# nikitakaraevv/ray-tracing-engine

Hardware: AMD Instinct MI355X
Metric: Mrays/s (primary+secondary) at 1024x1024/128spp path trace (higher is better)
Workload: dtype f32

## Files before the change

### include/rt_pixelmode.h

```cpp
#ifndef RT_PIXELMODE_H
#define RT_PIXELMODE_H

#include <stdint.h>
#include <string.h>

#if defined(__HIPCC__)
#define RT_HD __host__ __device__ inline
#else
#define RT_HD static inline
#endif

#define RT_STREAM_PIXEL 0u
#define RT_STREAM_PHOTON 1u
#define RT_STREAM_AO 2u
#define RT_STREAM_LENS 3u
#define RT_STREAM_SHUTTER 4u
#define RT_STREAM_PICK 5u

RT_HD uint64_t rt_mix64(uint64_t z) {
  z ^= z >> 30;
  z *= 0xbf58476d1ce4e5b9ull;
  z ^= z >> 27;
  z *= 0x94d049bb133111ebull;
  z ^= z >> 31;
// ... 19 lines not shown
  memcpy(&d, &u, 8);
  return d;
}

RT_HD double rt_pow2(double x) { return x * x; }
RT_HD double rt_pow5(double x) {
  double x2 = x * x;
  return (x2 * x2) * x;
}

#if defined(__HIP_DEVICE_COMPILE__)
RT_HD double rt_sqrt_d(double x) { return __dsqrt_rn(x); }
#else
RT_HD double rt_sqrt_d(double x) { return __builtin_sqrt(x); }
#endif

RT_HD double rt_asin_poly(double t) {
  const double pS0 = 1.66666666666666657415e-01, pS1 = -3.25565818622400915405e-01,
               pS2 = 2.01212532134862925881e-01, pS3 = -4.00555345006794114027e-02,
               pS4 = 7.91534994289814532176e-04, pS5 = 3.47933107596021167570e-05,
               qS1 = -2.40339491173441421878e+00, qS2 = 2.02094576023350569471e+00,
               qS3 = -6.88283971605453293030e-01, qS4 = 7.70381505559019352791e-02;
  double p = t * (pS0 + t * (pS1 + t * (pS2 + t * (pS3 + t * (pS4 + t * pS5)))));
  double q = 1.0 + t * (qS1 + t * (qS2 + t * (qS3 + t * qS4)));
  return p / q;
}

RT_HD double rt_asin(double x) {
  const double pio2_hi = 1.57079632679489655800e+00, pio2_lo = 6.12323399573676603587e-17,
               pio4_hi = 7.85398163397448278999e-01;
  double ax = x < 0.0 ? -x : x;
  if (!(ax <= 1.0)) return rt_u2d(0x7ff8000000000000ull);
  if (ax == 1.0) return x * pio2_hi + x * pio2_lo;
  if (ax < 0.5) {
    if (ax < 7.450580596923828125e-09) return x;
    return x + x * rt_asin_poly(x * x);
  }
  double w = 1.0 - ax;
  double t = w * 0.5;
  double r = rt_asin_poly(t);
  double s = rt_sqrt_d(t);
  double res;
  if (ax >= 0.975) {
    res = pio2_hi - (2.0 * (s + s * r) - pio2_lo);
  } else {
    double sh = rt_u2d(rt_d2u(s) & 0xffffffff00000000ull);
    double c = (t - sh * sh) / (s + sh);
    double p = 2.0 * s * r - (pio2_lo - 2.0 * c);
    double q = pio4_hi - 2.0 * sh;
    res = pio4_hi - (p - q);
  }
  return x < 0.0 ? -res : res;
}

RT_HD double rt_ksin(double r) {
  const double S1 = -1.66666666666666324348e-01, S2 = 8.33333333332248946124e-03,
               S3 = -1.98412698298579493134e-04, S4 = 2.75573137070700676789e-06,
               S5 = -2.50507602534068634195e-08, S6 = 1.58969099521155010221e-10;
  double z = r * r;
  double v = z * r;
  double p = S2 + z * (S3 + z * (S4 + z * (S5 + z * S6)));
  return r + v * (S1 + z * p);
}
RT_HD double rt_kcos(double r) {
  const double C1 = 4.16666666666666019037e-02, C2 = -1.38888888888741095749e-03,
               C3 = 2.48015872894767294178e-05, C4 = -2.75573143513906633035e-07,
               C5 = 2.08757232129817482790e-09, C6 = -1.13596475577881948265e-11;
  double z = r * r;
  double p = z * (C1 + z * (C2 + z * (C3 + z * (C4 + z * (C5 + z * C6)))));
  return 1.0 - (0.5 * z - z * p);
}
RT_HD double rt_reduce_pio2(float xf, int* quadrant) {
  const double invpio2 = 6.36619772367581382433e-01, pio2_1 = 1.57079632673412561417e+00,
// ... 43 lines not shown
```

### ray-tracing-engine_amd/csrc/rt_api.cpp

```cpp
#include <hip/hip_runtime.h>

#include <dlfcn.h>
#include <rccl/rccl.h>

#include <algorithm>
#include <chrono>
#include <cmath>
#include <map>
#include <memory>
#include <mutex>
#include <cstdarg>
#include <cstdio>
#include <cstdlib>
#include <cstring>
#include <initializer_list>
#include <string>
#include <thread>
#include <type_traits>
#include <vector>

#include "bvh_build.h"
#include "filters.h"
#include "rt_amd.h"
#include "rt_kernels.h"

namespace {

thread_local std::string g_err;

int fail(int code, const char* fmt, ...) {
  char buf[512];
  va_list ap;
  va_start(ap, fmt);
  vsnprintf(buf, sizeof buf, fmt, ap);
  va_end(ap);
  g_err = buf;
  return code;
}

#define HIP_TRY(expr)                                                                      \
  do {                                                                                     \
    hipError_t e_ = (expr);                                                                \
    if (e_ != hipSuccess) return fail(RT_ERR_HIP, "%s failed: %s", #expr, hipGetErrorString(e_)); \
  } while (0)

int select_device(int device) {
  int n = 0;
  hipError_t e = hipGetDeviceCount(&n);
  if (e != hipSuccess || n <= 0)
    return fail(RT_ERR_NO_DEVICE, "no HIP device available (%s); this library has no CPU path",
                e == hipSuccess ? "device count is 0" : hipGetErrorString(e));
  if (device < 0 || device >= n) return fail(RT_ERR_NO_DEVICE, "device %d out of range (0..%d)", device, n - 1);
  hipDeviceProp_t prop;
  HIP_TRY(hipGetDeviceProperties(&prop, device));
  if (strncmp(prop.gcnArchName, "gfx950", 6) != 0)
    return fail(RT_ERR_NO_DEVICE, "device %d is %s; kernels are built for gfx950 only", device, prop.gcnArchName);
  HIP_TRY(hipSetDevice(device));
// ... 120 lines not shown
    return RT_OK;
  }
};

struct StreamList {
  DevBuf<uint32_t> d;
  PinnedBuf<uint32_t> h;
  Event ready;
  hipStream_t on = nullptr;
  uint32_t n = 0;
};
int stream_upload(StreamList* L, const std::vector<uint32_t>& v, hipStream_t stream) {
  L->n = 0;
  if (L->d) {
    HIP_TRY(hipEventSynchronize(L->ready.get()));
    HIP_TRY(hipFree(L->d.release()));
  }
  L->h.reset();
  if (v.empty()) return RT_OK;
  HIP_TRY(dev_alloc(&L->d, v.size()));
  HIP_TRY(pinned_alloc(&L->h, v.size()));
  memcpy(L->h.get(), v.data(), v.size() * sizeof(uint32_t));
  if (!L->ready) HIP_TRY(make_event(&L->ready, hipEventDisableTiming));
  HIP_TRY(hipMemcpyAsync(L->d.get(), L->h.get(), v.size() * sizeof(uint32_t), hipMemcpyHostToDevice, stream));
  HIP_TRY(hipEventRecord(L->ready.get(), stream));
  L->on = stream, L->n = static_cast<uint32_t>(v.size());
  return RT_OK;
}
int use_on(const StreamList& L, hipStream_t stream) {
  if (L.d && stream != L.on) HIP_TRY(hipStreamWaitEvent(stream, L.ready.get(), 0));
  return RT_OK;
}

struct TileKey {
  uint32_t w = 0, h = 0, rank = 0, world = 0, tile = 0, sshift = 0;
  bool operator==(const TileKey& o) const {
    return w == o.w && h == o.h && rank == o.rank && world == o.world && tile == o.tile && sshift == o.sshift;
  }
};

void wave_tile_shape(uint32_t sshift, uint32_t& tw, uint32_t& th) {
  static const uint32_t W[7] = {8, 8, 4, 4, 2, 2, 1}, H[7] = {8, 4, 4, 2, 2, 1, 1};
  tw = W[sshift], th = H[sshift];
}

constexpr int kEventPairs = 256;

}

struct rt_ctx {
  int device = 0;
  rtk::DevScene S{};
  rtbvh::Built bvh;
  DevBuf<uint4> triShade, nodes, q8;
  DevBuf<float> vpos, vnrm;
  DevBuf<float4> tris, trisRef;
  DevBuf<rt_material> mats;
  DevBuf<rtd::DevMat> matsDev;
  DevBuf<rt_light> lights;
  DevBuf<uint32_t> meshTriBegin, meshVtxBegin;
  DevBuf<float4> nodesF;
  DevBuf<float4> phPos, phDir;
  DevBuf<uint4> phTopo;
  StreamList tiles;
  TileKey tileKey;
  DevBuf<unsigned long long> dCounters;
  DevBuf<uint32_t> dTileCounter;
  using GranList = StreamList;
  std::map<std::string, GranList> granules;
  rtk::WfArgs wf{};
  size_t wfCap = 0;
  DevBuf<char> wfBlock;
  uint32_t builder = RT_BVH_HOST;
  bool broken = false;
  uint32_t recipCheck = 0;
  uint32_t nodeFormat = RT_NODES_F16;
  float buildMs = 0.f;
  uint32_t numCUs = 0;
  Event ev[kEventPairs][2];
  int evUsed = 0;
  std::vector<rt_light> hostLights;
  uint32_t nMeshes = 0, nVertices = 0;
  uint32_t magRef = 0, magPos = 0, magNrm = 0;
  DevBuf<uint8_t> refitDepth;
  uint32_t refitMaxDepth = 0;
  uint32_t optLeafMax = 0, optBuilder = RT_BVH_AUTO, optNodeFormat = RT_NODES_AUTO;
  double costBuilt = 0.0;
  bool costBuiltValid = false;
  uint32_t refits = 0;
  DevBuf<double> dQuality;
  DevBuf<float> updPos, updNrm;
  DevBuf<uint32_t> dMag;
  DevBuf<float> restPos, restNrm;
  bool restValid = false;
  DevBuf<rt_mesh_transform> xfTable;
  DevBuf<uint16_t> skinBone;
  DevBuf<float> skinWeight;
  DevBuf<rt_mesh_transform> skinTable;
// ... 60 lines not shown
void install_photons(rt_ctx* c, DevBuf<float4> pos, DevBuf<float4> dir, DevBuf<uint4> topo, uint32_t n) {
  c->phPos = std::move(pos), c->phDir = std::move(dir), c->phTopo = std::move(topo);
  c->S.phPos = c->phPos.get(), c->S.phDir = c->phDir.get(), c->S.phTopo = c->phTopo.get(), c->S.n_photons = n;
}
uint32_t photons_per_light(uint32_t n_requested, uint32_t n_lights) {
  const float lightPdf = 1.f / static_cast<float>(n_lights);
  return static_cast<uint32_t>(static_cast<int>(static_cast<float>(static_cast<int>(n_requested)) * lightPdf));
}

uint32_t choose_sshift_px(const rt_ctx* c, const rt_params* p, uint64_t pixels, uint32_t spp_count, bool pick = false) {
  if (p->reserved[0]) {
    uint32_t s = 0;
    while ((1u << (s + 1)) <= p->reserved[0] && s < 6) ++s;
    return s;
  }
  const uint64_t target = 32ull * 256 * 16;
  uint32_t s = 0;
  while (s < 6 && (pixels << s) / 64 < target && (2u << s) <= spp_count) ++s;
  const bool pooled = !p->use_photons && p->accel != RT_ACCEL_BRUTE && (pick || c->S.n_lights <= 3u) && !(p->reserved[1] & 1u) &&
                      !(p->reserved[2] & 1u);
  if (pooled) {
    const uint32_t want = c->S.n_nodes > 65536u ? 6u : 4u;
    while (s < want && (2u << s) <= spp_count) ++s;
  }
  if (p->use_photons && p->accel != RT_ACCEL_BRUTE)
    while (s < 6u && (2u << s) <= spp_count) ++s;
  return s;
}
uint32_t choose_sshift(const rt_ctx* c, const rt_params* p, uint32_t spp_count, bool pick = false) {
  const uint64_t world = p->world ? p->world : 1;
  return choose_sshift_px(c, p, (uint64_t)p->width * p->height / world, spp_count, pick);
}

template <class F>
void owned_granules(uint32_t w, uint32_t h, uint32_t rank, uint32_t world, uint32_t tile, F f) {
  if (tile == 0) tile = 8;
  if (world == 0) world = 1;
  const uint32_t gx = (w + 7) / 8, gy = (h + 7) / 8;
  for (uint32_t y8 = 0; y8 < gy; ++y8)
    for (uint32_t x8 = 0; x8 < gx; ++x8)
      if (world <= 1 || (x8 * 8 / tile + y8 * 8 / tile) % world == rank) f(x8, y8);
}

TileKey tile_key(const rt_params* p, uint32_t sshift) {
  TileKey k;
  k.w = p->width, k.h = p->height, k.rank = p->rank, k.world = p->world ? p->world : 1;
  k.tile = p->tile ? p->tile : 8;
  k.sshift = sshift;
  return k;
}
std::vector<uint32_t> wave_tiles(const TileKey& k) {
  std::vector<uint32_t> tiles;
  uint32_t tw, th;
  wave_tile_shape(k.sshift, tw, th);
  owned_granules(k.w, k.h, k.rank, k.world, k.tile, [&](uint32_t x8, uint32_t y8) {
    for (uint32_t y = y8 * 8; y < y8 * 8 + 8 && y < k.h; y += th)
      for (uint32_t x = x8 * 8; x < x8 * 8 + 8 && x < k.w; x += tw) tiles.push_back(x | (y << 16));
  });
  return tiles;
}

int ensure_tiles(rt_ctx* c, const rt_params* p, uint32_t sshift, hipStream_t stream) {
  const TileKey k = tile_key(p, sshift);
  if (c->tiles.d && k == c->tileKey) return use_on(c->tiles, stream);
  const int rc = stream_upload(&c->tiles, wave_tiles(k), stream);
  if (rc != RT_OK) return rc;
  c->tileKey = k;
  return RT_OK;
}

int ensure_granules(rt_ctx* c, const rt_params* p, uint32_t rank, hipStream_t stream, const rt_ctx::GranList** out) {
  char key[96];
  snprintf(key, sizeof key, "%u.%u.%u.%u.%u", p->width, p->height, rank, p->world ? p->world : 1, p->tile ? p->tile : 8);
  auto it = c->granules.find(key);
  if (it == c->granules.end()) {
    std::vector<uint32_t> g;
    owned_granules(p->width, p->height, rank, p->world, p->tile, [&](uint32_t x8, uint32_t y8) { g.push_back(x8 | (y8 << 16)); });
    rt_ctx::GranList L;
    int rc = stream_upload(&L, g, stream);
    if (rc != RT_OK) return rc;
    it = c->granules.emplace(key, std::move(L)).first;
  } else {
    const int rc = use_on(it->second, stream);
    if (rc != RT_OK) return rc;
  }
  *out = &it->second;
  return RT_OK;
}

int check_params_shape(const rt_params* p) {
  if (p->width == 0 || p->height == 0 || p->width > 65535u || p->height > 65535u)
    return fail(RT_ERR_INVALID, "image size %ux%u out of range", p->width, p->height);
  if (p->spp == 0) return fail(RT_ERR_INVALID, "spp must be >= 1");
  if (p->mode != RT_MODE_RAY && p->mode != RT_MODE_PATH) return fail(RT_ERR_INVALID, "mode must be 0 or 1");
  if (p->rng_mode != RT_RNG_PIXEL)
    return fail(RT_ERR_UNSUPPORTED,
                "rng_mode legacy is one global serial engine (reference LightSource.h:6) and cannot run in "
                "parallel; the GPU path implements RT_RNG_PIXEL only");
  if (p->max_depth < 1 || p->max_depth > 3) return fail(RT_ERR_UNSUPPORTED, "max_depth must be in 1..3");
  if (p->world > 1 && p->rank >= p->world) return fail(RT_ERR_INVALID, "rank %u >= world %u", p->rank, p->world);
  if (p->tile % 8 != 0) return fail(RT_ERR_INVALID, "tile must be a multiple of 8");
// ... 110 lines not shown
    W.col = reinterpret_cast<float4*>(take(P * 48));
    W.org = reinterpret_cast<float4*>(take(P * 16)), W.dir = reinterpret_cast<float4*>(take(P * 16));
    W.nrm = reinterpret_cast<float4*>(take(P * 16)), W.pnt = reinterpret_cast<float4*>(take(P * 16));
    W.res = reinterpret_cast<uint2*>(take(P * 32)), W.key = reinterpret_cast<uint2*>(take(P * 8));
    W.rng = reinterpret_cast<uint32_t*>(take(P * 4));
    W.stripes = reinterpret_cast<unsigned long long*>(take(2048 * sizeof(unsigned long long)));
    const hipError_t he = hipMemsetAsync(W.stripes, 0, 2048 * sizeof(unsigned long long), stream);
    if (he != hipSuccess) {
      c->wfCap = 0;
      return fail(RT_ERR_HIP, "wavefront stripes reset failed: %s", hipGetErrorString(he));
    }
  }
  rtk::WfArgs W = c->wf;
  W.gran = G->d.get(), W.nGran = G->n, W.width = p->width, W.height = p->height, W.spp = p->spp, W.seed = p->seed;
  W.s0 = A.s0, W.s1 = A.s1, W.batch = (uint32_t)batch, W.nPaths = 0;
  *out = W;
  return RT_OK;
}

struct TileList {
  const uint32_t* tiles;
  uint32_t n, sshift;
  const uint32_t* tileView = nullptr;
  const rtk::ViewRec* views = nullptr;
  const rtk::ViewShutterRec* viewShutters = nullptr;
};

using FrameGen = rtk::FrameVariant;

int launch_frame(rt_ctx* c, const rt_params* p, float4* dAccum, hipStream_t stream, int* evIndex,
                 const TileList* own = nullptr, const FrameGen& gen = FrameGen()) {
  const SampleRange sr = sample_range(*p);
  const uint32_t sshift = own ? own->sshift : choose_sshift(c, p, sr.count, gen.kind == FrameGen::PICK);
  int rc = own ? RT_OK : ensure_tiles(c, p, sshift, stream);
  if (rc != RT_OK) return rc;
  rtk::RenderArgs A;
  A.sshift = sshift;
  wave_tile_shape(sshift, A.tileW, A.tileH);
  A.tiles = own ? own->tiles : c->tiles.d.get(), A.n_tiles = own ? own->n : c->tiles.n;
  A.tileView = own ? own->tileView : nullptr, A.views = own ? own->views : nullptr;
  A.viewShutters = own ? own->viewShutters : nullptr;
  A.width = p->width, A.height = p->height, A.spp = p->spp;
  A.s0 = sr.s0, A.s1 = sr.s1;
  A.mode = p->mode, A.max_depth = p->max_depth, A.seed = p->seed;
  A.k = p->k, A.photons_requested = p->photons_requested;
  static const bool noPool = getenv("RT_NO_POOL") != nullptr;
  A.flags = (noPool || (p->reserved[1] & 1u)) ? 0u : 1u;
  if (c->bvh.leafMax <= 2u) A.flags |= 2u;
  uint32_t levels = c->bvh.maxDepth > 1 ? c->bvh.maxDepth : 1;
  A.kd16 = 0;
  if (p->use_photons) {
    const KdStack ks = kd_stack(c->S.n_photons);
    A.kd16 = ks.kd16 ? 1u : 0u;
    levels = levels > ks.rows ? levels : ks.rows;
  }
  A.stackLevels = stack_levels(levels);
  A.tileCounter = c->dTileCounter.get(), A.numCUs = c->numCUs, A.waveWords = 0, A.tilesPerBlock = 1;
  const bool wavefront = (p->reserved[2] & 1u) && !p->use_photons && p->accel != RT_ACCEL_BRUTE && c->S.n_lights <= 3u;
  rtk::WfArgs W{};
  if (wavefront && (rc = wavefront_args(c, p, A, sr.count, stream, &W)) != RT_OK) return rc;
  return timed_launch(c, stream, evIndex, [&] {
    if (const FrameGen V = A.viewShutters ? FrameGen(FrameGen::VIEWS_SHUTTER) : gen) {
      hipError_t he = rtk::launch_render_variant(V, p->accel == RT_ACCEL_BRUTE, p->collect_stats != 0, c->S, A, dAccum,
                                                 c->dCounters.get(), stream);
      if (he != hipSuccess) return fail(RT_ERR_HIP, "%s render launch failed: %s", V.name(), hipGetErrorString(he));
    } else if (!wavefront) {
      hipError_t he = rtk::launch_render(p->accel == RT_ACCEL_BRUTE, p->use_photons != 0, p->collect_stats != 0, c->S, A,
                                         dAccum, c->dCounters.get(), stream);
      if (he != hipSuccess) return fail(RT_ERR_HIP, "render launch failed: %s", hipGetErrorString(he));
    } else if (W.nGran) {
      hipError_t hw = rtk::launch_wavefront(c->S, W, p->mode, p->max_depth, dAccum, c->dCounters.get(), c->dTileCounter.get(),
                                            A.stackLevels, c->numCUs, stream);
      if (hw != hipSuccess) return fail(RT_ERR_HIP, "wavefront launch failed: %s", hipGetErrorString(hw));
    }
    return (int)RT_OK;
  });
}

}

extern "C" {

int rt_abi_version(void) { return RT_ABI_VERSION; }
const char* rt_last_error(void) { return g_err.c_str(); }

}

namespace {
int create_ctx(const rt_scene_desc* sc, const rt_options* opt, const rtbvh::Built* prebuilt, rt_ctx** out);
}

// ... 3318 lines not shown
```

### ray-tracing-engine_amd/csrc/rt_kernels.h

```cpp
#pragma once

#include <hip/hip_runtime.h>
#include <stdint.h>

#include "bvh_build.h"
#include "rt_amd.h"
#include "rt_device.h"

#define RTK_KMAX 16

enum {
  RTK_CNT_CLOSEST = 0,
  RTK_CNT_SHADOW,
  RTK_CNT_KNN,
  RTK_CNT_NODES,
  RTK_CNT_TRIS,
  RTK_CNT_KD,
  RTK_CNT_WNODE,
  RTK_CNT_WLEAF,
  RTK_CNT_LWAIT,
  RTK_CNT_LIDLE,
  RTK_CNT_FRAMES,
  RTK_CNT_COUNT = 32
};
// ... 32 lines not shown
struct ViewRec {
  rt_camera cam;
  uint32_t seed;
  uint32_t accumOff;
  uint32_t pad[2];
};
static_assert(sizeof(ViewRec) == 64, "ViewRec is four 16-byte scalar loads");

struct ViewShutterRec {
  float d[12];
  float open, close;
  float aperture;
  float fs0, dfs;
  uint32_t pad[3];
};
static_assert(sizeof(ViewShutterRec) == 80 && sizeof(ViewShutterRec) % 16 == 0, "ViewShutterRec is five 16-byte scalar loads");

struct RenderArgs {
  const uint32_t* tiles;
  uint32_t n_tiles;
  uint32_t width, height, spp, s0, s1, mode, max_depth, seed, k, photons_requested;
  uint32_t flags;
  uint32_t stackLevels;
  uint32_t kd16;
  uint32_t sshift;
  uint32_t tileW, tileH;
  uint32_t tilesPerBlock;
  uint32_t* tileCounter;
  uint32_t waveWords;
  uint32_t numCUs;
  const uint32_t* tileView;
  const ViewRec* views;
  const ViewShutterRec* viewShutters;
};

hipError_t launch_render(bool brute_force, bool photon, bool stats, const DevScene& S, const RenderArgs& A,
                         float4* accum, unsigned long long* counters, hipStream_t stream);
hipError_t launch_resolve(uint32_t n_pixels, uint32_t spp, const float4* accum, const float* bg, float* out,
                          hipStream_t stream);
struct WfArgs {
  const uint32_t* gran;
  uint32_t nGran, width, height, spp, seed;
  uint32_t s0, s1;
  uint32_t batch;
  uint32_t nPaths;
  uint32_t* rng;
  float4 *org, *dir;
  uint2* key;
  float4 *nrm, *pnt;
  float4* col;
  float4 *rayO, *rayD;
  uint2* res;
  unsigned long long* stripes;
};
hipError_t launch_wavefront(const DevScene& S, const WfArgs& W, uint32_t mode, uint32_t maxDepth, float4* accum,
                            unsigned long long* counters, uint32_t* queueCounter, uint32_t stackLevels, uint32_t numCUs,
                            hipStream_t stream);
struct TexDesc;
struct TexRec;
struct AovArgs {
  float *albedo, *normal, *position, *depth;
  uint32_t *hits, *mesh, *tri;
  uint32_t width, height, spp, seed, s0, s1;
  const ViewRec* views = nullptr;
  uint32_t tilesPerView = 0;
  const float* vcol = nullptr;
  const float* texUv = nullptr;
  const uint32_t* texMesh = nullptr;
// ... 168 lines not shown
```

### ray-tracing-engine_amd/csrc/rt_kernels.hip

```cpp
#include <hip/hip_runtime.h>

#include <cstdio>
#include <cstdlib>
#include <type_traits>

#include "bvh_build.h"
#include "filters.h"
#include "rt_device.h"
#include "rt_kernels.h"

using namespace rtd;

namespace rtk {

constexpr int BLOCK = 64;
constexpr int STACK = rtbvh::kMaxDepth;
constexpr int KMAX = RTK_KMAX;

struct Lds {
  uint32_t* stack;
  uint2* heap;
};

#ifdef RT_PHASE_TIMING
// ... 1092 lines not shown
  wave_sync();
  if (owner) {
    const uint32_t cnt = A.s1 - base < S_ ? A.s1 - base : S_;
#pragma unroll
    for (int g = 0; g < RT_LIGHT_GROUPS_MAX; ++g) {
      if ((uint32_t)g < G.n) {
        float4 s = accum[g * slice + pix];
        for (uint32_t jj = 0; jj < cnt; jj++) {
          const uint32_t q = jj * P_ + pl;
          s.x += ex[(3 * g + 0) * 64 + q], s.y += ex[(3 * g + 1) * 64 + q], s.z += ex[(3 * g + 2) * 64 + q];
          s.w += ex[HIT + q];
        }
        accum[g * slice + pix] = s;
      }
    }
  }
  wave_sync();
}

struct NoRec {};
template <int LTV>
using frame_rec_t = std::conditional_t<(LTV & LT_LENS) != 0, LensRec,
                    std::conditional_t<(LTV & LT_LIGHTS) != 0, LightGroupsRec,
                    std::conditional_t<(LTV & LT_PICK) != 0, PickRec,
                    std::conditional_t<(LTV & LT_VCOL) != 0, VColRec,
                    std::conditional_t<(LTV & LT_TEX) != 0, TexRec,
                    std::conditional_t<(LTV & LT_SHUTTER) != 0 && (LTV & LT_VIEWS) == 0, ShutterRec, NoRec>>>>>>;
template <int LTV>
constexpr const frame_rec_t<LTV>* no_record() {
  static_assert(std::is_same_v<frame_rec_t<LTV>, NoRec>, "this variant's instances pass their record to render_tile");
  return nullptr;
}

template <bool BRUTE, bool PHOTON, bool POOLED, bool STATS, int LTV, class HP = Heap>
RT_DEV void render_tile(const DevScene& S, const RenderArgs& A, float4* __restrict__ accum, const Lds& L, uint32_t* pool,
                        float* ex, uint32_t wave, LaneStats& st, const frame_rec_t<LTV>* rec = no_record<LTV>(),
                        float* park = nullptr) {
  constexpr int LT = LTV & ~(LT_VIEWS | LT_LENS | LT_SHUTTER | LT_LIGHTS | LT_PICK | LT_VCOL | LT_TEX);
  constexpr bool VIEWS = (LTV & LT_VIEWS) != 0;
  constexpr bool LENS = (LTV & LT_LENS) != 0;
  constexpr bool SHUTTER = (LTV & LT_SHUTTER) != 0;
  constexpr bool LIGHTS = (LTV & LT_LIGHTS) != 0;
  constexpr bool PICK = (LTV & LT_PICK) != 0;
  constexpr bool VCOL = (LTV & LT_VCOL) != 0;
  constexpr bool TEX = (LTV & LT_TEX) != 0;
  static_assert(!VCOL || (!VIEWS && !LENS && !SHUTTER && !LIGHTS && !PICK && !PHOTON), "vertex colours go with the plain frame only");
  static_assert(!TEX || (!VIEWS && !LENS && !SHUTTER && !LIGHTS && !PICK && !VCOL && !PHOTON), "textures go with the plain frame only");
  static_assert(!LIGHTS || (!VIEWS && !LENS && !SHUTTER && !PHOTON), "light groups go with the plain frame only");
  static_assert(!PICK || (!VIEWS && !LENS && !SHUTTER && !LIGHTS && !PHOTON), "light picks go with the plain frame only");
  static_assert(!LENS || !VIEWS, "no multi-view lens frames");
  static_assert(!SHUTTER || !LENS, "the shutter's lens is its own: LT_SHUTTER does not go with LT_LENS");
  constexpr bool FR = (LT & LT_FASTDET) != 0;
  const uint32_t lane = threadIdx.x & 63u;
  const uint32_t tile = A.tiles[wave];
  rt_camera cam;
  uint32_t seed = A.seed;
  ShutterRec vsh;
  if constexpr (VIEWS) {
    typedef const __attribute__((address_space(4))) uint32_t* const_u32_ptr;
    typedef const __attribute__((address_space(4))) ViewRec* const_view_ptr;
    typedef const __attribute__((address_space(4))) ViewShutterRec* const_shutter_ptr;
    const uint32_t view = ((const_u32_ptr)A.tileView)[wave];
    const const_view_ptr R = (const_view_ptr)A.views + view;
    for (int j = 0; j < 3; ++j)
      cam.position[j] = R->cam.position[j], cam.lower_left[j] = R->cam.lower_left[j],
      cam.horizontal[j] = R->cam.horizontal[j], cam.vertical[j] = R->cam.vertical[j];
    seed = R->seed;
    accum += R->accumOff;
    if constexpr (SHUTTER) {
      const const_shutter_ptr Q = (const_shutter_ptr)A.viewShutters + view;
      for (int j = 0; j < 12; ++j) vsh.d[j] = Q->d[j];
      vsh.open = Q->open, vsh.close = Q->close, vsh.aperture = Q->aperture, vsh.fs0 = Q->fs0, vsh.dfs = Q->dfs;
    }
  }
  const uint32_t S_ = 1u << A.sshift, P_ = 64u >> A.sshift;
  const uint32_t pl = lane & (P_ - 1u), sj = lane >> (6u - A.sshift);
  const uint32_t wsh = (uint32_t)__builtin_ctz(A.tileW);
  const uint32_t px = (tile & 0xffffu) + (pl & (A.tileW - 1u)), py = (tile >> 16) + (pl >> wsh);
  const bool inImage = px < A.width && py < A.height;
  const bool owner = inImage && sj == 0;
  const uint32_t pix = inImage ? py * A.width + px : 0u;
  float4 sum = owner ? accum[pix] : make_float4(0.f, 0.f, 0.f, 0.f);
  constexpr bool pooled = POOLED;
  const int nvert = A.mode == RT_MODE_PATH ? (int)A.max_depth : 1;
  for (uint32_t base = A.s0; base < A.s1; base += S_) {
    const uint32_t i = base + sj;
    const bool active = inImage && i < A.s1;
    Rng g{rt_stream_seed(VIEWS ? seed : A.seed, RT_STREAM_PIXEL, pix, i)};
    float sx, sy;
    jitter_sample(g, (int)i, (int)A.spp, sx, sy);
    f3 o, d;
    const float cu = ((float)px + sx) / (float)A.width, cv = 1.f - ((float)py + sy) / (float)A.height;
    if constexpr (VIEWS && SHUTTER) shutter_ray(cam, vsh, seed, pix, i, cu, cv, o, d);
    else if constexpr (VIEWS) camera_ray<FR>(cam, cu, cv, o, d);
    else if constexpr (LENS) {
      if (rec->aperture > 0.f) lens_ray(S.cam, *rec, rt_stream_seed(A.seed, RT_STREAM_LENS, pix, i), cu, cv, o, d);
      else camera_ray<FR>(S.cam, cu, cv, o, d);
    } else if constexpr (SHUTTER) shutter_ray(S.cam, *rec, A.seed, pix, i, cu, cv, o, d);
    else camera_ray<FR>(S.cam, cu, cv, o, d);
    f3 c0 = mk(0.f, 0.f, 0.f), c1 = c0, c2 = c0;
    GroupCols g0, g1, g2, gv;
    if constexpr (LIGHTS) group_cols_zero(g0), group_cols_zero(g1), group_cols_zero(g2);
    bool primary = true, alive = active;
    Picks pk{0u, 0u, 0u};
    if constexpr (PICK) pk = draw_picks(*rec, A.seed, pix, i);
    if constexpr (pooled) {
      HitRec h;
      if (alive) st.closest++;
      const bool hit0 = cast<false, false, STATS, LT>(S, alive, o, d, L.stack, h, st);
      if (alive && !hit0) primary = false, alive = false;
      for (int depth = 0; depth < nvert; depth++) {
// ... 71 lines not shown
        if (alive)
          c = shade_direct_seq<BRUTE, STATS, false, NoPick, VColKd>(S, g, d, h, L.stack, nrm, pt, st, nullptr, nullptr, NoPick(),
                                                                    VColKd{vertex_kd(S, rec->vcol, S.triShade[h.id], h.u, h.v), park});
      } else if constexpr (TEX) {
        if (alive)
          c = shade_direct_seq<BRUTE, STATS, false, NoPick, VColKd>(S, g, d, h, L.stack, nrm, pt, st, nullptr, nullptr, NoPick(),
                                                                    VColKd{tex_kd(S, *rec, S.triShade[h.id], h.u, h.v), park});
      } else {
        if (alive) c = shade_direct_seq<BRUTE, STATS>(S, g, d, h, L.stack, nrm, pt, st);
      }
      if (alive) {
        if (depth == 0) c0 = c;
        else if (depth == 1) c1 = c;
        else c2 = c;
        if constexpr (LIGHTS) {
          if (depth == 0) g0 = gv;
          else if (depth == 1) g1 = gv;
          else g2 = gv;
        }
      }
      if (A.mode != RT_MODE_PATH) break;
      if (alive) {
        d = hemisphere_sample(g, nrm);
        o = pt;
      }
    }
    PH(PH_VSETUP);
    if constexpr (LIGHTS) {
      group_samples_add(A, *rec, accum, ex, g0, g1, g2, primary, active, owner, pix, pl, base);
      continue;
    }
    const f3 total = c0 + (c1 + (c2 + mk(0.f, 0.f, 0.f)));
    const float r0 = clamp01(total.x), r1 = clamp01(total.y), r2 = clamp01(total.z);
    if (A.sshift == 0) {
      if (active) {
        sum.x += r0, sum.y += r1, sum.z += r2;
        if (primary) sum.w += 1.f;
      }
    } else {
      ex[lane] = r0, ex[64 + lane] = r1, ex[128 + lane] = r2, ex[192 + lane] = primary ? 1.f : 0.f;
      wave_sync();
      if (owner) {
        const uint32_t cnt = A.s1 - base < S_ ? A.s1 - base : S_;
        for (uint32_t jj = 0; jj < cnt; jj++) {
          const uint32_t q = jj * P_ + pl;
          sum.x += ex[q], sum.y += ex[64 + q], sum.z += ex[128 + q];
          sum.w += ex[192 + q];
        }
      }
      wave_sync();
    }
    PH(PH_ACCUM);
  }
  if constexpr (LIGHTS) return;
  if (owner) accum[pix] = sum;
}

template <bool BRUTE, bool PHOTON, bool POOLED, bool STATS, int MINW, int LTV = LT_NONE>
__global__ __launch_bounds__(BLOCK, MINW) void k_render(DevScene S, RenderArgs A, float4* __restrict__ accum,
                                                  unsigned long long* __restrict__ counters) {
  static_assert(BLOCK == 64, "one wave per workgroup");
  static_assert(!POOLED || (!BRUTE && !PHOTON), "the vertex pool serves BVH direct lighting");
  uint32_t* lds = g_lds;
  const Lds L = carve_lds<PHOTON>(lds, A.stackLevels, A.k);
  uint32_t* pool = lds + (A.stackLevels + (PHOTON ? 2 * A.k : 0)) * BLOCK;
  float* ex = reinterpret_cast<float*>(POOLED ? pool : lds);
  LaneStats st;
  const uint32_t t0 = blockIdx.x * A.tilesPerBlock, t1 = min(A.n_tiles, t0 + A.tilesPerBlock);
  for (uint32_t t = t0; t < t1; ++t) render_tile<BRUTE, PHOTON, POOLED, STATS, LTV>(S, A, accum, L, pool, ex, t, st);
  if (STATS) flush_stats(st, counters, true);
  else flush_stats_striped(st, counters);
}

template <bool BRUTE, bool STATS, int MINW, int HL, int LTV = LT_NONE>
__global__ __launch_bounds__(BLOCK, MINW) void k_render_wide(DevScene S, RenderArgs A, float4* __restrict__ accum,
                                                          unsigned long long* __restrict__ counters) {
  uint32_t* lds = g_lds;
  const Lds L = carve_lds<true>(lds, A.stackLevels, A.k);
  float* ex = reinterpret_cast<float*>(lds);
  LaneStats st;
  const uint32_t t0 = blockIdx.x * A.tilesPerBlock, t1 = min(A.n_tiles, t0 + A.tilesPerBlock);
  for (uint32_t t = t0; t < t1; ++t)
    render_tile<BRUTE, true, false, STATS, LTV, WideHeap<HL>>(S, A, accum, L, nullptr, ex, t, st);
  if (STATS) flush_stats(st, counters, true);
  else flush_stats_striped(st, counters);
}

template <bool STATS, int LT>
RT_DEV void persist_body(const DevScene& S, const RenderArgs& A, float4* __restrict__ accum, unsigned long long* __restrict__ counters) {
  const uint32_t lane = threadIdx.x & 63u, wv = threadIdx.x >> 6;
  {
    uint4* dst = reinterpret_cast<uint4*>(g_lds);
    for (uint32_t i = threadIdx.x; i < 2u * S.topK; i += blockDim.x) dst[i] = S.nodes[i];
  }
  __syncthreads();
  uint32_t* mine = g_lds + 8u * S.topK + wv * A.waveWords;
  Lds L = carve_lds<false>(mine, A.stackLevels, 0);
  uint32_t* pool = mine + A.stackLevels * BLOCK;
  float* ex = reinterpret_cast<float*>((LT & LT_COMPACT3) ? mine : pool);
  LaneStats st;
#ifdef RT_PHASE_TIMING
  if (threadIdx.x < 24) g_phAcc[threadIdx.x] = 0;
  if (threadIdx.x == 0) g_phT0 = __builtin_amdgcn_s_memtime();
  __syncthreads();
#endif
  for (;;) {
    uint32_t t = 0;
    if (lane == 0) t = atomicAdd(A.tileCounter, 1u);
    t = (uint32_t)__builtin_amdgcn_readfirstlane((int)t);
    if (t >= A.n_tiles) break;
    render_tile<false, false, true, STATS, LT>(S, A, accum, L, pool, ex, t, st);
  }
#ifdef RT_PHASE_TIMING
  __syncthreads();
  if (threadIdx.x < PH_COUNT) atomicAdd(&counters[16 + threadIdx.x], g_phAcc[threadIdx.x]);
#endif
  flush_stats(st, counters, STATS);
}

template <bool STATS, int LT>
__global__ __launch_bounds__(1024) void k_render_persist(DevScene S, RenderArgs A, float4* __restrict__ accum,
                                                         unsigned long long* __restrict__ counters) {
  persist_body<STATS, LT>(S, A, accum, counters);
}
template <bool STATS, int LT>
__global__ __launch_bounds__(256, 5) void k_render_persist5(DevScene S, RenderArgs A, float4* __restrict__ accum,
                                                            unsigned long long* __restrict__ counters) {
  persist_body<STATS, LT>(S, A, accum, counters);
}

__global__ void k_resolve(uint32_t n_pixels, float spp, const float4* __restrict__ accum,
                          const float* __restrict__ bg, float* __restrict__ out) {
  const uint32_t i = blockIdx.x * blockDim.x + threadIdx.x;
  if (i >= n_pixels) return;
  const float4 a = accum[i];
  const float miss = (float)((int)spp - (int)a.w);
  out[3 * i + 0] = a.x / spp + bg[3 * i + 0] * miss / spp;
  out[3 * i + 1] = a.y / spp + bg[3 * i + 1] * miss / spp;
  out[3 * i + 2] = a.z / spp + bg[3 * i + 2] * miss / spp;
}

constexpr int STREAM_CHUNK = 2048;
template <int LT>
__global__ __launch_bounds__(1024, 8) void k_trace_stream(DevScene S, const float4* __restrict__ rayO,
                                                          const float4* __restrict__ rayD, uint32_t n,
                                                          uint2* __restrict__ res, uint32_t* __restrict__ counter,
                                                          uint32_t stackLevels) {
  const uint32_t lane = threadIdx.x & 63u, wv = threadIdx.x >> 6;
  if (LT != LT_NONE) {
    uint4* dst = reinterpret_cast<uint4*>(g_lds);
    for (uint32_t i = threadIdx.x; i < 2u * S.topK; i += blockDim.x) dst[i] = S.nodes[i];
    __syncthreads();
  }
  uint32_t* stack = g_lds + 8u * S.topK + wv * stackLevels * BLOCK + lane;
  Trav<TRAV_MIXED, LT> T;
  T.idle(stack);
// ... 394 lines not shown
  const size_t ldsBytes = 4u * (size_t)(A.stackLevels + heap_rows(hl, A.k)) * BLOCK;
  if (A.k > (uint32_t)RT_KNN_KMAX || ldsBytes > 4u * (size_t)rtbvh::kLdsWordsPerCU) return hipErrorInvalidValue;
  RenderArgs A1 = A;
  A1.tilesPerBlock = 1u;
#define RT_LAUNCH_WIDE1(ST, MW, HLV, LTV)                                                                             \
  do {                                                                                                                \
    static unsigned long long done = 0;                                                                               \
    if (!allow_big_lds(&k_render_wide<BRUTE, ST, MW, HLV, LTV>, done)) return hipErrorInvalidConfiguration;            \
    knn_report(k_render_wide<BRUTE, ST, MW, HLV, LTV>, "k_render_wide", HLV, A.k, ldsBytes);                          \
    hipLaunchKernelGGL((k_render_wide<BRUTE, ST, MW, HLV, LTV>), dim3(A.n_tiles), dim3(BLOCK), ldsBytes, stream, S, A1, \
                       accum, counters);                                                                              \
  } while (0)
#define RT_LAUNCH_WIDE(ST, MW, HLV)                        \
  do {                                                     \
    if (A.tileView) RT_LAUNCH_WIDE1(ST, MW, HLV, LT_VIEWS); \
    else RT_LAUNCH_WIDE1(ST, MW, HLV, LT_NONE);            \
  } while (0)
#define RT_LAUNCH_WIDE_HL(ST, MW)                                   \
  do {                                                              \
    if (hl == HEAP_SPLIT16) RT_LAUNCH_WIDE(ST, MW, HEAP_SPLIT16);   \
    else RT_LAUNCH_WIDE(ST, MW, HEAP_WIDE8);                        \
  } while (0)
  if (stats) RT_LAUNCH_WIDE_HL(true, 1);
  else {
    RT_LAUNCH_WIDE_HL(false, MINW_WIDE);
    hipLaunchKernelGGL(k_fold_stripes, dim3(1), dim3(1024), 0, stream, counters);
  }
#undef RT_LAUNCH_WIDE_HL
#undef RT_LAUNCH_WIDE
#undef RT_LAUNCH_WIDE1
  return hipGetLastError();
}

template <bool BRUTE, bool PHOTON, bool POOLED>
static hipError_t launch_render2(bool stats, const DevScene& S, const RenderArgs& A, float4* accum,
                                 unsigned long long* counters, hipStream_t stream) {
  const uint32_t blocks = A.n_tiles;
  if (blocks == 0) return hipSuccess;
  static const bool noPersist = getenv("RT_NO_PERSIST") != nullptr;
  if (POOLED && !noPersist && A.tileCounter && A.numCUs) {
    const PersistPlan P = plan_persist(S, A);
    if (P.waves) {
      DevScene S2 = S;
      RenderArgs A2 = A;
      S2.topK = P.topK, A2.waveWords = P.waveWords;
      hipError_t e = hipMemsetAsync(A.tileCounter, 0, sizeof(uint32_t), stream);
      if (e != hipSuccess) return e;
      const uint32_t perCU = P.waves;
      const uint32_t slots = P.compact == 3 ? 5u * A.numCUs : A.numCUs;
      const uint32_t wgs = (blocks + perCU - 1) / perCU < slots ? (blocks + perCU - 1) / perCU : slots;
#define RT_LAUNCH_PERSIST1(ST, LTV)                                                                         \
  do {                                                                                                      \
    static unsigned long long done = 0;                                                                     \
    if (!allow_big_lds(&k_render_persist<ST, LTV>, done)) return hipErrorInvalidConfiguration;              \
    hipLaunchKernelGGL((k_render_persist<ST, LTV>), dim3(wgs), dim3(64u * P.waves), P.ldsBytes, stream, S2, \
                       A2, accum, counters);                                                                \
  } while (0)
#define RT_LAUNCH_PERSIST(ST, LTV)                                \
  do {                                                            \
    if (A.tileView) RT_LAUNCH_PERSIST1(ST, (LTV) | LT_VIEWS);     \
    else RT_LAUNCH_PERSIST1(ST, LTV);                             \
  } while (0)
#define RT_LAUNCH_EITHER(LTV)                                    \
  do {                                                           \
    if (stats || S.slowRecip) RT_LAUNCH_PERSIST(true, LTV);      \
    else RT_LAUNCH_PERSIST(false, (LTV) | LT_FASTDET);           \
  } while (0)
      const char* const leaf2Env = getenv("RT_LEAF2");
      const bool leaf2 = (A.flags & 2u) && !(leaf2Env && atoi(leaf2Env) == 0) && !stats && !S.slowRecip && !A.tileView;
#define RT_LAUNCH_LEAF2(LTV)                                             \
  do {                                                                   \
    if (leaf2) RT_LAUNCH_PERSIST1(false, (LTV) | LT_FASTDET | LT_LEAF2); \
    else RT_LAUNCH_EITHER(LTV);                                          \
// ... 27 lines not shown
      else RT_LAUNCH_EITHER(LT_NONE | LT_NOPRIO);
#undef RT_LAUNCH_LEAF2
#undef RT_LAUNCH_EITHER
#undef RT_LAUNCH_PERSIST
#undef RT_LAUNCH_PERSIST1
      return hipGetLastError();
    }
  }
  if (PHOTON && A.k > (uint32_t)KMAX) return launch_render_wide<BRUTE>(stats, S, A, accum, counters, stream);
  const uint32_t rows = A.stackLevels + (PHOTON ? 2 * A.k : 0);
  const size_t ldsBytes = 4u * ((rows < 4u ? 4u : rows) * BLOCK + (POOLED ? VP_WORDS : 0));
  RenderArgs A1 = A;
  A1.tilesPerBlock = 1u;
  const uint32_t nBlocks = blocks;
  constexpr int MINW = PHOTON ? 5 : 4;
  if (PHOTON) knn_report(stats ? k_render<BRUTE, PHOTON, POOLED, true, 1> : k_render<BRUTE, PHOTON, POOLED, false, MINW>,
                         "k_render", -1, A.k, ldsBytes);
  if (stats) {
    if (A.tileView) hipLaunchKernelGGL((k_render<BRUTE, PHOTON, POOLED, true, 1, LT_VIEWS>), dim3(nBlocks), dim3(BLOCK), ldsBytes, stream, S, A1, accum, counters);
    else hipLaunchKernelGGL((k_render<BRUTE, PHOTON, POOLED, true, 1>), dim3(nBlocks), dim3(BLOCK), ldsBytes, stream, S, A1, accum, counters);
  } else {
    if (A.tileView) hipLaunchKernelGGL((k_render<BRUTE, PHOTON, POOLED, false, MINW, LT_VIEWS>), dim3(nBlocks), dim3(BLOCK), ldsBytes, stream, S, A1, accum, counters);
    else hipLaunchKernelGGL((k_render<BRUTE, PHOTON, POOLED, false, MINW>), dim3(nBlocks), dim3(BLOCK), ldsBytes, stream, S, A1, accum, counters);
    hipLaunchKernelGGL(k_fold_stripes, dim3(1), dim3(1024), 0, stream, counters);
  }
  return hipGetLastError();
}

hipError_t launch_render(bool brute_force, bool photon, bool stats, const DevScene& S, const RenderArgs& A,
                         float4* accum, unsigned long long* counters, hipStream_t stream) {
  if (brute_force) return photon ? launch_render2<true, true, false>(stats, S, A, accum, counters, stream)
                                 : launch_render2<true, false, false>(stats, S, A, accum, counters, stream);
  if (photon) return launch_render2<false, true, false>(stats, S, A, accum, counters, stream);
  if ((A.flags & 1u) && S.n_lights <= (uint32_t)POOL_L) return launch_render2<false, false, true>(stats, S, A, accum, counters, stream);
  return launch_render2<false, false, false>(stats, S, A, accum, counters, stream);
}

hipError_t launch_resolve(uint32_t n_pixels, uint32_t spp, const float4* accum, const float* bg, float* out,
                          hipStream_t stream) {
  if (n_pixels == 0) return hipSuccess;
  hipLaunchKernelGGL(k_resolve, dim3((n_pixels + 255) / 256), dim3(256), 0, stream, n_pixels, (float)spp, accum,
                     bg, out);
  return hipGetLastError();
}

hipError_t launch_trace_stream(const DevScene& S, const float4* rayO, const float4* rayD, uint32_t n, uint2* res,
                               uint32_t* counter, uint32_t stackLevels, uint32_t numCUs, hipStream_t stream) {
  if (n == 0) return hipSuccess;
  hipError_t e = hipMemsetAsync(counter, 0, sizeof(uint32_t), stream);
  if (e != hipSuccess) return e;
  const uint32_t total = 160u * 1024u / 4u / 2u - 32u;
  uint32_t wpw = 16u;
  while (wpw > 1u && wpw * stackLevels * BLOCK > total) --wpw;
  const uint32_t stackWords = wpw * stackLevels * BLOCK;
  static const int kEnv = getenv("RT_STREAM_TOPK") ? atoi(getenv("RT_STREAM_TOPK")) : -1;
  DevScene S2 = S;
  S2.topK = 0;
  if (stackWords > total) return hipErrorInvalidValue;
  if (stackWords + 8u * S.n_nodes <= total) S2.topK = S.n_nodes;
  if (kEnv >= 0) S2.topK = (uint32_t)kEnv < S2.topK ? (uint32_t)kEnv : S2.topK;
  const uint32_t ldsBytes = 4u * (8u * S2.topK + stackWords);
  const uint32_t waves = (n + 63u) / 64u;
  uint32_t wgs = (waves + wpw - 1u) / wpw;
  static const uint32_t perCU = getenv("RT_STREAM_WGS") ? (uint32_t)atoi(getenv("RT_STREAM_WGS")) : 2u;
  wgs = wgs < perCU * numCUs ? wgs : perCU * numCUs;
  if (S2.topK >= S.n_nodes && S2.topK) {
    static unsigned long long done = 0;
// ... 108 lines not shown
```

Measured before the change: 33090.

## Split tail wave tiles into finer sample-split tiles to balance persistent render

The last N tiles of the persistent pooled render queue (by default one per resident wave) are split into smaller pixel tiles with more samples per pixel per wave. The goal is to shorten the load-imbalance tail at the end of the frame, when few waves still hold large tiles. The kernel template gains a FINE path that switches sshift and tile width per tile index, which adds a branch and some register pressure. Separately, rt_asin now evaluates its polynomial before the small/large branch, so both ranges share one call site and divergence drops.

Result: faster. 33440, median of 6 (+1.1%).

```diff
diff --git a/include/rt_pixelmode.h b/include/rt_pixelmode.h
--- a/include/rt_pixelmode.h
+++ b/include/rt_pixelmode.h
@@ -75,13 +75,14 @@
   double ax = x < 0.0 ? -x : x;
   if (!(ax <= 1.0)) return rt_u2d(0x7ff8000000000000ull);
   if (ax == 1.0) return x * pio2_hi + x * pio2_lo;
-  if (ax < 0.5) {
+  const int small = ax < 0.5;
+  double w = 1.0 - ax;
+  double t = small ? x * x : w * 0.5;
+  double r = rt_asin_poly(t);
+  if (small) {
     if (ax < 7.450580596923828125e-09) return x;
-    return x + x * rt_asin_poly(x * x);
+    return x + x * r;
   }
-  double w = 1.0 - ax;
-  double t = w * 0.5;
-  double r = rt_asin_poly(t);
   double s = rt_sqrt_d(t);
   double res;
   if (ax >= 0.975) {
diff --git a/ray-tracing-engine_amd/csrc/rt_api.cpp b/ray-tracing-engine_amd/csrc/rt_api.cpp
--- a/ray-tracing-engine_amd/csrc/rt_api.cpp
+++ b/ray-tracing-engine_amd/csrc/rt_api.cpp
@@ -23,6 +23,7 @@
 #include "filters.h"
 #include "rt_amd.h"
 #include "rt_kernels.h"
+#include "wave_tiles.h"
 
 namespace {
 
@@ -209,17 +210,10 @@
   return RT_OK;
 }
 
-struct TileKey {
-  uint32_t w = 0, h = 0, rank = 0, world = 0, tile = 0, sshift = 0;
-  bool operator==(const TileKey& o) const {
-    return w == o.w && h == o.h && rank == o.rank && world == o.world && tile == o.tile && sshift == o.sshift;
-  }
-};
-
-void wave_tile_shape(uint32_t sshift, uint32_t& tw, uint32_t& th) {
-  static const uint32_t W[7] = {8, 8, 4, 4, 2, 2, 1}, H[7] = {8, 4, 4, 2, 2, 1, 1};
-  tw = W[sshift], th = H[sshift];
-}
+using rtl::owned_granules;
+using rtl::TileKey;
+using rtl::wave_tile_shape;
+using rtl::wave_tiles;
 
 constexpr int kEventPairs = 256;
 
@@ -241,6 +235,7 @@
   DevBuf<uint4> phTopo;
   StreamList tiles;
   TileKey tileKey;
+  uint32_t tilesFineFrom = 0;
   DevBuf<unsigned long long> dCounters;
   DevBuf<uint32_t> dTileCounter;
   using GranList = StreamList;
@@ -367,16 +362,6 @@
   return choose_sshift_px(c, p, (uint64_t)p->width * p->height / world, spp_count, pick);
 }
 
-template <class F>
-void owned_granules(uint32_t w, uint32_t h, uint32_t rank, uint32_t world, uint32_t tile, F f) {
-  if (tile == 0) tile = 8;
-  if (world == 0) world = 1;
-  const uint32_t gx = (w + 7) / 8, gy = (h + 7) / 8;
-  for (uint32_t y8 = 0; y8 < gy; ++y8)
-    for (uint32_t x8 = 0; x8 < gx; ++x8)
-      if (world <= 1 || (x8 * 8 / tile + y8 * 8 / tile) % world == rank) f(x8, y8);
-}
-
 TileKey tile_key(const rt_params* p, uint32_t sshift) {
   TileKey k;
   k.w = p->width, k.h = p->height, k.rank = p->rank, k.world = p->world ? p->world : 1;
@@ -384,24 +369,25 @@
   k.sshift = sshift;
   return k;
 }
-std::vector<uint32_t> wave_tiles(const TileKey& k) {
-  std::vector<uint32_t> tiles;
-  uint32_t tw, th;
-  wave_tile_shape(k.sshift, tw, th);
-  owned_granules(k.w, k.h, k.rank, k.world, k.tile, [&](uint32_t x8, uint32_t y8) {
-    for (uint32_t y = y8 * 8; y < y8 * 8 + 8 && y < k.h; y += th)
-      for (uint32_t x = x8 * 8; x < x8 * 8 + 8 && x < k.w; x += tw) tiles.push_back(x | (y << 16));
-  });
-  return tiles;
-}
-
-int ensure_tiles(rt_ctx* c, const rt_params* p, uint32_t sshift, hipStream_t stream) {
-  const TileKey k = tile_key(p, sshift);
+
+int ensure_tiles(rt_ctx* c, const rt_params* p, uint32_t sshift, hipStream_t stream, uint32_t fine = 0, uint32_t sshiftFine = 0) {
+  TileKey k = tile_key(p, sshift);
+  if (fine && sshiftFine > sshift) k.fine = fine, k.sshiftFine = sshiftFine;
   if (c->tiles.d && k == c->tileKey) return use_on(c->tiles, stream);
-  const int rc = stream_upload(&c->tiles, wave_tiles(k), stream);
-  if (rc != RT_OK) return rc;
-  c->tileKey = k;
-  return RT_OK;
+  uint32_t from = 0;
+  const int rc = stream_upload(&c->tiles, wave_tiles(k, &from), stream);
+  if (rc != RT_OK) return rc;
+  c->tileKey = k, c->tilesFineFrom = from;
+  return RT_OK;
+}
+
+uint32_t fine_tail_tiles(uint32_t waves) {
+  if (!waves) return 0;
+  const char* const e = getenv("RT_FINE_TAIL");
+  if (!e || !*e) return waves;
+  if (!strcmp(e, "all")) return ~0u;
+  const long n = atol(e);
+  return n <= 0 ? 0u : (uint32_t)std::min<long>(n, 0x7fffffff);
 }
 
 int ensure_granules(rt_ctx* c, const rt_params* p, uint32_t rank, hipStream_t stream, const rt_ctx::GranList** out) {
@@ -578,12 +564,10 @@
                  const TileList* own = nullptr, const FrameGen& gen = FrameGen()) {
   const SampleRange sr = sample_range(*p);
   const uint32_t sshift = own ? own->sshift : choose_sshift(c, p, sr.count, gen.kind == FrameGen::PICK);
-  int rc = own ? RT_OK : ensure_tiles(c, p, sshift, stream);
-  if (rc != RT_OK) return rc;
+  int rc = RT_OK;
   rtk::RenderArgs A;
   A.sshift = sshift;
   wave_tile_shape(sshift, A.tileW, A.tileH);
-  A.tiles = own ? own->tiles : c->tiles.d.get(), A.n_tiles = own ? own->n : c->tiles.n;
   A.tileView = own ? own->tileView : nullptr, A.views = own ? own->views : nullptr;
   A.viewShutters = own ? own->viewShutters : nullptr;
   A.width = p->width, A.height = p->height, A.spp = p->spp;
@@ -603,6 +587,13 @@
   A.stackLevels = stack_levels(levels);
   A.tileCounter = c->dTileCounter.get(), A.numCUs = c->numCUs, A.waveWords = 0, A.tilesPerBlock = 1;
   const bool wavefront = (p->reserved[2] & 1u) && !p->use_photons && p->accel != RT_ACCEL_BRUTE && c->S.n_lights <= 3u;
+  uint32_t fine = 0, sshiftFine = std::min(6u, sshift + 2u);
+  while (sshiftFine > sshift && (1u << sshiftFine) > sr.count) --sshiftFine;
+  if (!own && !gen && !wavefront)
+    fine = fine_tail_tiles(rtk::persist_fine_waves(p->accel == RT_ACCEL_BRUTE, p->use_photons != 0, c->S, A));
+  if (!own && (rc = ensure_tiles(c, p, sshift, stream, fine, sshiftFine)) != RT_OK) return rc;
+  A.tiles = own ? own->tiles : c->tiles.d.get(), A.n_tiles = own ? own->n : c->tiles.n;
+  A.fineFrom = own ? A.n_tiles : c->tilesFineFrom, A.sshiftFine = own ? sshift : c->tileKey.sshiftFine;
   rtk::WfArgs W{};
   if (wavefront && (rc = wavefront_args(c, p, A, sr.count, stream, &W)) != RT_OK) return rc;
   return timed_launch(c, stream, evIndex, [&] {
diff --git a/ray-tracing-engine_amd/csrc/rt_kernels.h b/ray-tracing-engine_amd/csrc/rt_kernels.h
--- a/ray-tracing-engine_amd/csrc/rt_kernels.h
+++ b/ray-tracing-engine_amd/csrc/rt_kernels.h
@@ -88,8 +88,10 @@
   const uint32_t* tileView;
   const ViewRec* views;
   const ViewShutterRec* viewShutters;
-};
-
+  uint32_t fineFrom = ~0u, sshiftFine = 0;
+};
+
+uint32_t persist_fine_waves(bool brute_force, bool photon, const DevScene& S, const RenderArgs& A);
 hipError_t launch_render(bool brute_force, bool photon, bool stats, const DevScene& S, const RenderArgs& A,
                          float4* accum, unsigned long long* counters, hipStream_t stream);
 hipError_t launch_resolve(uint32_t n_pixels, uint32_t spp, const float4* accum, const float* bg, float* out,
diff --git a/ray-tracing-engine_amd/csrc/rt_kernels.hip b/ray-tracing-engine_amd/csrc/rt_kernels.hip
--- a/ray-tracing-engine_amd/csrc/rt_kernels.hip
+++ b/ray-tracing-engine_amd/csrc/rt_kernels.hip
@@ -1148,7 +1148,7 @@
   return nullptr;
 }
 
-template <bool BRUTE, bool PHOTON, bool POOLED, bool STATS, int LTV, class HP = Heap>
+template <bool BRUTE, bool PHOTON, bool POOLED, bool STATS, int LTV, class HP = Heap, bool FINE = false>
 RT_DEV void render_tile(const DevScene& S, const RenderArgs& A, float4* __restrict__ accum, const Lds& L, uint32_t* pool,
                         float* ex, uint32_t wave, LaneStats& st, const frame_rec_t<LTV>* rec = no_record<LTV>(),
                         float* park = nullptr) {
@@ -1189,10 +1189,17 @@
       vsh.open = Q->open, vsh.close = Q->close, vsh.aperture = Q->aperture, vsh.fs0 = Q->fs0, vsh.dfs = Q->dfs;
     }
   }
-  const uint32_t S_ = 1u << A.sshift, P_ = 64u >> A.sshift;
-  const uint32_t pl = lane & (P_ - 1u), sj = lane >> (6u - A.sshift);
-  const uint32_t wsh = (uint32_t)__builtin_ctz(A.tileW);
-  const uint32_t px = (tile & 0xffffu) + (pl & (A.tileW - 1u)), py = (tile >> 16) + (pl >> wsh);
+  uint32_t sshift = A.sshift, tileW = A.tileW;
+  if constexpr (FINE) {
+    static_assert(POOLED && LTV == LT, "the fine tail goes with the plain pooled frame only");
+    if (wave >= A.fineFrom) {
+      sshift = A.sshiftFine, tileW = 8u >> (A.sshiftFine >> 1);
+    }
+  }
+  const uint32_t S_ = 1u << sshift, P_ = 64u >> sshift;
+  const uint32_t pl = lane & (P_ - 1u), sj = lane >> (6u - sshift);
+  const uint32_t wsh = (uint32_t)__builtin_ctz(tileW);
+  const uint32_t px = (tile & 0xffffu) + (pl & (tileW - 1u)), py = (tile >> 16) + (pl >> wsh);
   const bool inImage = px < A.width && py < A.height;
   const bool owner = inImage && sj == 0;
   const uint32_t pix = inImage ? py * A.width + px : 0u;
@@ -1330,7 +1337,7 @@
     }
     const f3 total = c0 + (c1 + (c2 + mk(0.f, 0.f, 0.f)));
     const float r0 = clamp01(total.x), r1 = clamp01(total.y), r2 = clamp01(total.z);
-    if (A.sshift == 0) {
+    if (sshift == 0) {
       if (active) {
         sum.x += r0, sum.y += r1, sum.z += r2;
         if (primary) sum.w += 1.f;
@@ -1384,7 +1391,7 @@
   else flush_stats_striped(st, counters);
 }
 
-template <bool STATS, int LT>
+template <bool STATS, int LT, bool FINE = false>
 RT_DEV void persist_body(const DevScene& S, const RenderArgs& A, float4* __restrict__ accum, unsigned long long* __restrict__ counters) {
   const uint32_t lane = threadIdx.x & 63u, wv = threadIdx.x >> 6;
   {
@@ -1407,7 +1414,7 @@
     if (lane == 0) t = atomicAdd(A.tileCounter, 1u);
     t = (uint32_t)__builtin_amdgcn_readfirstlane((int)t);
     if (t >= A.n_tiles) break;
-    render_tile<false, false, true, STATS, LT>(S, A, accum, L, pool, ex, t, st);
+    render_tile<false, false, true, STATS, LT, Heap, FINE>(S, A, accum, L, pool, ex, t, st);
   }
 #ifdef RT_PHASE_TIMING
   __syncthreads();
@@ -1419,7 +1426,7 @@
 template <bool STATS, int LT>
 __global__ __launch_bounds__(1024) void k_render_persist(DevScene S, RenderArgs A, float4* __restrict__ accum,
                                                          unsigned long long* __restrict__ counters) {
-  persist_body<STATS, LT>(S, A, accum, counters);
+  persist_body<STATS, LT, (LT & LT_VIEWS) == 0>(S, A, accum, counters);
 }
 template <bool STATS, int LT>
 __global__ __launch_bounds__(256, 5) void k_render_persist5(DevScene S, RenderArgs A, float4* __restrict__ accum,
@@ -1880,13 +1887,25 @@
   return hipGetLastError();
 }
 
+static bool persist_wanted(const RenderArgs& A) {
+  static const bool noPersist = getenv("RT_NO_PERSIST") != nullptr;
+  return !noPersist && A.tileCounter && A.numCUs;
+}
+static bool pool_wanted(const DevScene& S, const RenderArgs& A) { return (A.flags & 1u) && S.n_lights <= (uint32_t)POOL_L; }
+
+uint32_t persist_fine_waves(bool brute_force, bool photon, const DevScene& S, const RenderArgs& A) {
+  if (brute_force || photon || !pool_wanted(S, A) || !persist_wanted(A) || A.tileView) return 0;
+  const PersistPlan P = plan_persist(S, A);
+  return P.compact == 3 ? 0u : P.waves * A.numCUs;
+}
+
 template <bool BRUTE, bool PHOTON, bool POOLED>
 static hipError_t launch_render2(bool stats, const DevScene& S, const RenderArgs& A, float4* accum,
                                  unsigned long long* counters, hipStream_t stream) {
   const uint32_t blocks = A.n_tiles;
   if (blocks == 0) return hipSuccess;
-  static const bool noPersist = getenv("RT_NO_PERSIST") != nullptr;
-  if (POOLED && !noPersist && A.tileCounter && A.numCUs) {
+  if (A.fineFrom < A.n_tiles && !(POOLED && persist_fine_waves(false, false, S, A))) return hipErrorInvalidValue;
+  if (POOLED && persist_wanted(A)) {
     const PersistPlan P = plan_persist(S, A);
     if (P.waves) {
       DevScene S2 = S;
@@ -1980,7 +1999,7 @@
   if (brute_force) return photon ? launch_render2<true, true, false>(stats, S, A, accum, counters, stream)
                                  : launch_render2<true, false, false>(stats, S, A, accum, counters, stream);
   if (photon) return launch_render2<false, true, false>(stats, S, A, accum, counters, stream);
-  if ((A.flags & 1u) && S.n_lights <= (uint32_t)POOL_L) return launch_render2<false, false, true>(stats, S, A, accum, counters, stream);
+  if (pool_wanted(S, A)) return launch_render2<false, false, true>(stats, S, A, accum, counters, stream);
   return launch_render2<false, false, false>(stats, S, A, accum, counters, stream);
 }
 
diff --git a/ray-tracing-engine_amd/csrc/wave_tiles.h b/ray-tracing-engine_amd/csrc/wave_tiles.h
--- /dev/null
+++ b/ray-tracing-engine_amd/csrc/wave_tiles.h
@@ -0,0 +1,57 @@
+#pragma once
+#include <algorithm>
+#include <cstdint>
+#include <vector>
+
+namespace rtl {
+
+struct TileKey {
+  uint32_t w = 0, h = 0, rank = 0, world = 0, tile = 0, sshift = 0;
+  uint32_t fine = 0, sshiftFine = 0;
+  bool operator==(const TileKey& o) const {
+    return w == o.w && h == o.h && rank == o.rank && world == o.world && tile == o.tile && sshift == o.sshift &&
+           fine == o.fine && sshiftFine == o.sshiftFine;
+  }
+};
+
+inline void wave_tile_shape(uint32_t sshift, uint32_t& tw, uint32_t& th) {
+  static const uint32_t W[7] = {8, 8, 4, 4, 2, 2, 1}, H[7] = {8, 4, 4, 2, 2, 1, 1};
+  tw = W[sshift], th = H[sshift];
+}
+
+template <class F>
+void owned_granules(uint32_t w, uint32_t h, uint32_t rank, uint32_t world, uint32_t tile, F f) {
+  if (tile == 0) tile = 8;
+  if (world == 0) world = 1;
+  const uint32_t gx = (w + 7) / 8, gy = (h + 7) / 8;
+  for (uint32_t y8 = 0; y8 < gy; ++y8)
+    for (uint32_t x8 = 0; x8 < gx; ++x8)
+      if (world <= 1 || (x8 * 8 / tile + y8 * 8 / tile) % world == rank) f(x8, y8);
+}
+
+inline std::vector<uint32_t> wave_tiles(const TileKey& k, uint32_t* fineFrom = nullptr) {
+  std::vector<uint32_t> tiles;
+  uint32_t tw, th;
+  wave_tile_shape(k.sshift, tw, th);
+  owned_granules(k.w, k.h, k.rank, k.world, k.tile, [&](uint32_t x8, uint32_t y8) {
+    for (uint32_t y = y8 * 8; y < y8 * 8 + 8 && y < k.h; y += th)
+      for (uint32_t x = x8 * 8; x < x8 * 8 + 8 && x < k.w; x += tw) tiles.push_back(x | (y << 16));
+  });
+  uint32_t from = (uint32_t)tiles.size();
+  if (k.fine && k.sshiftFine > k.sshift) {
+    const uint32_t f = std::min<uint32_t>(k.fine, from);
+    const std::vector<uint32_t> split(tiles.end() - f, tiles.end());
+    tiles.resize(from -= f);
+    uint32_t fw, fh;
+    wave_tile_shape(k.sshiftFine, fw, fh);
+    for (const uint32_t t : split) {
+      const uint32_t x0 = t & 0xffffu, y0 = t >> 16;
+      for (uint32_t y = y0; y < y0 + th && y < k.h; y += fh)
+        for (uint32_t x = x0; x < x0 + tw && x < k.w; x += fw) tiles.push_back(x | (y << 16));
+    }
+  }
+  if (fineFrom) *fineFrom = from;
+  return tiles;
+}
+
+}
```
